# kywind/real2sim-eval

Hardware: AMD Instinct MI355X
Metric: sim env-steps/sec (phys+render) per node at 32 envs (higher is better)
Workload: dtype f32

## Files before the change

### real2sim-eval_amd/csrc/physics_substep.h

```cpp

typedef unsigned v4u __attribute__((ext_vector_type(4)));
constexpr unsigned PF_SENT = 0x7fc5e7a1u;
constexpr int PF_LINE = 128;
constexpr int PF_AUX_STORE = 16;
constexpr int PF_AUX_LOAD = 16 | (int)0x80000000;
__device__ __forceinline__ void resident_fault(const PhysDev& p, int code, int item, int k, unsigned a, unsigned b, unsigned c, unsigned d, unsigned e2, unsigned f)
{
    if (!p.fault) return;
    if (atomicCAS(p.fault, 0, code) == 0) {
        int* w = p.fault + 3;
        w[0] = code; w[1] = item; w[2] = k; w[3] = (int)a; w[4] = (int)b; w[5] = (int)c; w[6] = (int)d; w[7] = (int)e2; w[8] = (int)f;
    }
}
__device__ __forceinline__ bool pf_pending(v2f a) { return __float_as_uint(a.x) == PF_SENT && __float_as_uint(a.y) == PF_SENT; }
__device__ __forceinline__ void pf_mark(StateM s, size_t i)
{
    const v2f w = {__uint_as_float(PF_SENT), __uint_as_float(PF_SENT)};
    s.p[st_at(s.n, i, 0)] = w; s.p[st_at(s.n, i, 1)] = w; s.p[st_at(s.n, i, 2)] = w;
}
__device__ __forceinline__ void pf_store(const PhysDev& p, size_t ei, f3 x, f3 v, unsigned tag)
{
    const __amdgpu_buffer_rsrc_t r = __builtin_amdgcn_make_buffer_rsrc(p.pf_res, 0, 0x7fffffff, 0x00020000);
    const unsigned off = (unsigned)ei * (unsigned)PF_LINE;
    const v4u w0 = {__float_as_uint(x.x), tag, __float_as_uint(x.y), tag}, w1 = {__float_as_uint(x.z), tag, __float_as_uint(v.z), tag},
              w2 = {__float_as_uint(v.x), tag, __float_as_uint(v.y), tag};
    __builtin_amdgcn_raw_buffer_store_b128(w0, r, off, 0, PF_AUX_STORE);
    __builtin_amdgcn_raw_buffer_store_b128(w1, r, off + 16u, 0, PF_AUX_STORE);
    __builtin_amdgcn_raw_buffer_store_b128(w2, r, off + 32u, 0, PF_AUX_STORE);
}
__device__ __forceinline__ void pf_wait(const PhysDev& p, size_t ei, int step, int item, v2f& a, v2f& b, v2f& c)
{
    const __amdgpu_buffer_rsrc_t r = __builtin_amdgcn_make_buffer_rsrc(p.pf_res, 0, 0x7fffffff, 0x00020000);
    const unsigned off = (unsigned)ei * (unsigned)PF_LINE, tag = (unsigned)step;
    for (unsigned spins = 0;; ++spins) {
        const v4u d0 = __builtin_amdgcn_raw_buffer_load_b128(r, off, 0, PF_AUX_LOAD), d1 = __builtin_amdgcn_raw_buffer_load_b128(r, off + 16u, 0, PF_AUX_LOAD),
                  d2 = __builtin_amdgcn_raw_buffer_load_b128(r, off + 32u, 0, PF_AUX_LOAD);
        if (d0.y == tag && d0.w == tag && d1.y == tag && d1.w == tag && d2.y == tag && d2.w == tag) {
            a = (v2f){__uint_as_float(d0.x), __uint_as_float(d0.z)}; b = (v2f){__uint_as_float(d1.x), __uint_as_float(d1.z)};
            c = (v2f){__uint_as_float(d2.x), __uint_as_float(d2.z)};
            return;
        }
        if (spins >= p.spin_limit) {
            resident_fault(p, 6, item, step, (unsigned)ei, d0.y, d0.w, d1.y, d2.y, spins);
            a = (v2f){0.f, 0.f}; b = a; c = a;
            return;
        }
        __builtin_amdgcn_s_sleep(2);
    }
}

#pragma clang fp contract(fast)

__device__ __forceinline__ void spring_term(v2f xy, float zj, v2f vxy, float vzj, f3 xi, f3 vi, float k, float a, float dashpot,
                                            v2f& fxy, float& fz)
{
    const v2f dxy = xy - (v2f){xi.x, xi.y};
    const float dz = zj - xi.z;
    const float d2 = fmaf(dxy.x, dxy.x, fmaf(dxy.y, dxy.y, fmaf(dz, dz, 1e-30f)));
    const float rinv = __builtin_amdgcn_rsqf(d2);
    const v2f dvxy = vxy - (v2f){vi.x, vi.y};
    const float dvz = vzj - vi.z;
    const float t = fmaf(dvxy.x, dxy.x, fmaf(dvxy.y, dxy.y, dvz * dz));
    const float sc = fmaf(dashpot * (rinv * rinv), t, fmaf(-k, rinv, a));
    fxy += dxy * sc;
    fz = fmaf(dz, sc, fz);
}

template <int RCAP> __device__ __forceinline__ constexpr int PLANE1() { return RCAP * 8 + 8; }
template <int RCAP> __device__ __forceinline__ constexpr int PLANE2() { return 2 * (RCAP * 8 + 8); }

struct AdjGroup {
    uint2 idx;
    float4 k, a;
};
__device__ __forceinline__ AdjGroup adj_load(const PhysDev& p, int row, int lane)
{
    typedef unsigned v2u __attribute__((ext_vector_type(2)));
    typedef float v4f __attribute__((ext_vector_type(4)));
    const __amdgpu_buffer_rsrc_t ri = __builtin_amdgcn_make_buffer_rsrc((void*)p.adj_idx, 0, 0x7fffffff, 0x00020000);
    const __amdgpu_buffer_rsrc_t rk = __builtin_amdgcn_make_buffer_rsrc((void*)p.adj_k, 0, 0x7fffffff, 0x00020000);
    const __amdgpu_buffer_rsrc_t ra = __builtin_amdgcn_make_buffer_rsrc((void*)p.adj_ir, 0, 0x7fffffff, 0x00020000);
    const v2u i2 = __builtin_amdgcn_raw_buffer_load_b64(ri, (unsigned)lane * 8u, row * 8, 0);
    const v4f k4 = __builtin_amdgcn_raw_buffer_load_b128(rk, (unsigned)lane * 16u, row * 16, 0);
    const v4f a4 = __builtin_amdgcn_raw_buffer_load_b128(ra, (unsigned)lane * 16u, row * 16, 0);
    AdjGroup g;
    g.idx = make_uint2(i2.x, i2.y); g.k = make_float4(k4.x, k4.y, k4.z, k4.w); g.a = make_float4(a4.x, a4.y, a4.z, a4.w);
    return g;
}

template <int RCAP>
__device__ __forceinline__ void spring_group(const PhysDev& p, const AdjGroup& g, const __attribute__((address_space(3))) char* win, f3 xi,
                                             f3 vi, v2f& fxy, float& fz)
{
    typedef __attribute__((address_space(3))) const v2f lds_f2;
    const unsigned off[GROUP] = {g.idx.x & 0xffffu, g.idx.x >> 16, g.idx.y & 0xffffu, g.idx.y >> 16};
    const float k[GROUP] = {g.k.x, g.k.y, g.k.z, g.k.w};
    const float a[GROUP] = {g.a.x, g.a.y, g.a.z, g.a.w};
#pragma unroll
    for (int u = 0; u < GROUP; ++u) {
#ifdef R2S_WIN16
        typedef float v4f_ __attribute__((ext_vector_type(4)));
        typedef __attribute__((address_space(3))) const v4f_ lds_f4;
        const v4f_ xz = *(lds_f4*)(win + 2u * off[u]);
        const v2f vxy = *(lds_f2*)(win + off[u] + 2 * (RCAP * 8 + 8));
        spring_term((v2f){xz.x, xz.y}, xz.z, vxy, xz.w, xi, vi, k[u], a[u], p.dashpot, fxy, fz);
#else
        const v2f xy = *(lds_f2*)(win + off[u]);
        const v2f zz = *(lds_f2*)(win + off[u] + PLANE1<RCAP>());
        const v2f vxy = *(lds_f2*)(win + off[u] + PLANE2<RCAP>());
        spring_term(xy, zz.x, vxy, zz.y, xi, vi, k[u], a[u], p.dashpot, fxy, fz);
#endif
    }
}

template <int RCAP>
__device__ __forceinline__ f3 spring_force_lds(const PhysDev& p, const StateC xv,
                                               const __attribute__((address_space(3))) char* win, size_t env_base, int sl, int ln, f3 xi,
                                               f3 vi, int srow, int ngroups, AdjGroup g0, int pf_step = -1)
{
    v2f fxy = {0.f, 0.f};
    float fz = 0.f;
    AdjGroup a = g0, b = g0;
    int g = 0;
    for (; g + 2 <= ngroups; g += 2) {
        b = adj_load(p, srow + (g + 1) * SLICE, ln);
        spring_group<RCAP>(p, a, win, xi, vi, fxy, fz);
        a = adj_load(p, srow + min(g + 2, ngroups - 1) * SLICE, ln);
        spring_group<RCAP>(p, b, win, xi, vi, fxy, fz);
    }
    if (g < ngroups) spring_group<RCAP>(p, a, win, xi, vi, fxy, fz);
    const int4* __restrict__ ra = p.radj + p.rslice_off[sl] + ln;
    const int rdeg = p.rslice_deg[sl];
    for (int n = 0; n < rdeg; ++n) {
        const int4 en = ra[n * SLICE];
        const size_t gi = env_base + (size_t)en.x;
        v2f jxy = xv.p[st_at(xv.n, gi, 0)], jz = xv.p[st_at(xv.n, gi, 1)], jv = xv.p[st_at(xv.n, gi, 2)];
        if (pf_step >= 0 && pf_pending(jxy)) pf_wait(p, gi, pf_step, -1, jxy, jz, jv);
        spring_term(jxy, jz.x, jv, jz.y, xi, vi, __int_as_float(en.y), __int_as_float(en.z), p.dashpot, fxy, fz);
    }
    return {fxy.x, fxy.y, fz};
}

#pragma clang fp contract(off)

__device__ __forceinline__ float mesh_margin(const PhysDev& p, int m)
{
    return (p.mesh_kind[m] & 2) ? MESH_MAX_DIST : ((m < p.n_dyn_mesh && !p.use_pusher) ? 0.005f : 0.001f);
}
__device__ __forceinline__ bool mesh_need(const PhysDev& p, int e, int step, f3 next_x, float pad, bool& near, const float* staged = nullptr)
{
    bool need = false;
    near = false;
    for (int m = 0; m < p.n_mesh; ++m) {
        const float* bb = staged ? staged + 6 * m
                        : m < p.n_dyn_mesh ? p.aabb_dyn + (((size_t)e * p.n_sub + step) * p.n_dyn_mesh + m) * 6
                                           : p.aabb_static + ((size_t)e * (p.n_mesh - p.n_dyn_mesh) + (m - p.n_dyn_mesh)) * 6;
        const float mg = mesh_margin(p, m) + pad;
        const float d2 = box_dist2(next_x, bb);
        need = need || d2 < mg * mg * 1.0001f;
        near = near || d2 < (mg + NEAR_PAD) * (mg + NEAR_PAD);
    }
    return need;
}

constexpr int RES_MAX_MESH = 4;
constexpr float RES_RANGE_PAD = 0.002f;
struct ResidentIO {
    bool srv_on, srv_need;
    const float* step_boxes;
    f3 x, v;
    const float* boxes;
};
__device__ __forceinline__ bool resident_in_range(const ResidentIO& io, f3 next_x, bool fin)
{
    if (__builtin_amdgcn_ballot_w64(fin && box_dist2(next_x, io.boxes) < io.boxes[6]) == 0ull) return false;
    bool any = false;
#pragma unroll
    for (int m = 0; m < RES_MAX_MESH; ++m) any = any || box_dist2(next_x, io.boxes + 8 + 8 * m) < io.boxes[8 + 8 * m + 6];
    return __builtin_amdgcn_ballot_w64(fin && any) != 0ull;
}

__device__ __forceinline__ int mesh_rec_reserve(const PhysDev& p, int e, int step)
{
    int slot;
    {
        const unsigned long long act = __builtin_amdgcn_ballot_w64(true);
        const int e0 = __builtin_amdgcn_readfirstlane(e);
        if (__builtin_amdgcn_ballot_w64(e != e0) == 0ull) {
            const int rank = (int)__builtin_amdgcn_mbcnt_hi((unsigned)(act >> 32), __builtin_amdgcn_mbcnt_lo((unsigned)act, 0u));
            int base = 0;
            if (rank == 0) base = atomicAdd(p.rec_cnt + (size_t)e0 * p.n_sub + step, (int)__builtin_popcountll(act));
            slot = __builtin_amdgcn_readfirstlane(base) + rank;
        } else
            slot = atomicAdd(p.rec_cnt + (size_t)e * p.n_sub + step, 1);
    }
    return slot;
}
__device__ __forceinline__ void mesh_rec_write(const PhysDev& p, int e, int step, int slot, int i, int ncand, f3 x0, f3 v)
{
    int4* r = p.mesh_rec + 2 * (par_off(p, step) + (size_t)e * p.N + slot);
    const int hint = p.mq_hint ? p.mq_hint[(size_t)e * p.N + i] : -1;
    r[0] = make_int4(ncand | ((hint + 1) << 19), ncand > 0 ? (i | (int)0x80000000) : i, __float_as_int(x0.x), __float_as_int(x0.y));
    r[1] = make_int4(__float_as_int(x0.z), __float_as_int(v.x), __float_as_int(v.y), __float_as_int(v.z));
}
__device__ __forceinline__ bool mesh_rec_push(const PhysDev& p, int e, int step, int i, int ncand, f3 x0, f3 v)
{
    const int slot = mesh_rec_reserve(p, e, step);
    if (slot >= p.N) return false;
    mesh_rec_write(p, e, step, slot, i, ncand, x0, v);
    return true;
}

template <int MESH, bool MAIN = false, int NEED = 0, bool KEEP = false, bool QUAD = false, bool PFOUT = false>
__device__ __forceinline__ bool finish_wave(const PhysDev& p, int e, int i, size_t eb, int step, int write_forces, f3 x0, f3 v, bool fin,
                                            const StateM xv_out, const TriRegs* tr, QShare* qs, int* qpar, BlkAux* xf0, bool store, ResidentIO* keep R2S_QP_PARAM)
{
    f3 x = x0;
    if (MESH) {
        f3 vin = v;
        f3 next_x = x0 + vin * p.dt;
        f3 next_v = vin;
        bool in_range = true;
        if (KEEP && keep->boxes) in_range = resident_in_range(*keep, next_x, fin);
      if (in_range) {
        bool need = false, near = false;
        if (NEED == 1) need = fin;
        else if (NEED == 0 && fin) need = mesh_need(p, e, step, next_x, 0.f, near, KEEP ? keep->step_boxes : nullptr);
        if (MAIN) {
            const unsigned long long nm = __builtin_amdgcn_ballot_w64(near);
            if (nm && (int)(threadIdx.x & 63) == __builtin_ctzll(nm)) p.mesh_cnt[p.n_sub] = 1;
            const unsigned long long qm = __builtin_amdgcn_ballot_w64(need);
            if (qm && (int)(threadIdx.x & 63) == __builtin_ctzll(qm)) p.fault[1] = 1;
            if (MESH == 2) {
                if (need && mesh_rec_push(p, e, step, i, 0, x0, v)) { fin = false; need = false; }
            } else if (need && p.mesh_defer && p.mesh_rec) {
                if (mesh_rec_push(p, e, step, i, 0, x0, v)) { fin = false; need = false; }
            } else if (need && p.mesh_defer) {
                const int slot = atomicAdd(p.mesh_cnt + step, 1);
                if (slot < p.mesh_cap) {
                    const size_t po = par_off(p, step);
                    p.vdef[po + eb + i] = make_float4(v.x, v.y, v.z, 0.f);
                    p.xbc[po + eb + i] = make_float4(x0.x, x0.y, x0.z, 0.f);
                    p.mesh_list[po + slot] = make_int2(e, i);
                    fin = false;
                    need = false;
                }
            } else if (KEEP && need && keep->srv_on) {
                keep->srv_need = true;
                fin = false;
                need = false;
            }
        }
        constexpr bool IN_PLACE = !(MAIN && MESH == 2) && NEED != 2;
        MeshHit q = {false, 0.f, 0, mk(0.f, 0.f, 0.f), 0, 0};
        if (IN_PLACE)
            q = MESH == 3 ? mesh_query_regs<QUAD>(*tr, mk(bcast(next_x.x, 0), bcast(next_x.y, 0), bcast(next_x.z, 0)), bcasti((int)need, 0) != 0, *qs, *qpar)
              : MESH == 2 ? mesh_query_block(p, step, mk(bcast(next_x.x, 0), bcast(next_x.y, 0), bcast(next_x.z, 0)), e,
                                             bcasti((int)need, 0) != 0, xf0->hint, *qs, *qpar, *xf0 R2S_QP_ARG)
                          : mesh_query_lane(p, e, step, next_x, need);
        R2S_QSTAMP();
        bool requery = false;
        f3 normal = mk(0.f, 0.f, 0.f), v_normal = mk(0.f, 0.f, 0.f), v_normal_new = mk(0.f, 0.f, 0.f);
        float margin = 0.f;
        bool hit = false;
        if (q.result) {
            int is_gripper;
            const int mm = MESH >= 2 ? q.mm : p.mesh_map[q.face];
            if (!p.use_pusher) is_gripper = mm == 0 ? 1 : (mm == 1 ? 2 : 0);
            else is_gripper = mm >= 0 ? 1 : 0;
            f3 delta = next_x - q.pt;
            float dist = len(delta) * q.sign;
            margin = (is_gripper >= 1 && !p.use_pusher) ? 0.005f : 0.001f;
            float err = dist - margin;
            if (err < 0.f) {
                hit = true;
                normal = normalize0(delta) * q.sign;
                f3 rdv = mk(0.f, 0.f, 0.f);
                float ce, cf;
                if (is_gripper >= 1) {
                    const f3 ctr = MESH == 3 ? tr->ctr : ld3(p.interp_center, (size_t)e * p.n_sub + step);
                    const f3 om = MESH == 3 ? tr->om : ld3(p.dyn_omega, e);
                    const f3 dv = MESH == 3 ? (is_gripper == 1 ? tr->dv0 : tr->dv1) : ld3(p.dyn_vel, (size_t)e * 2 + (is_gripper == 1 ? 0 : 1));
                    rdv = dv + cross(om, x0 - ctr);
                    vin = vin - rdv;
                    ce = p.cee; cf = p.cef;
                } else {
                    ce = p.ce; cf = p.cf;
                }
                v_normal = normal * dot(vin, normal);
                const f3 v_tao = vin - v_normal;
                const float vnl = len(v_normal);
                const float vtl = fmaxf(len(v_tao), 1e-6f);
                v_normal_new = v_normal * (-ce);
                const float a = fmaxf(0.f, 1.f - cf * (1.f + ce) * vnl / vtl);
                next_v = v_normal_new + v_tao * a;
                if (is_gripper >= 1) {
                    next_v = next_v + rdv;
                    next_x = x0 + next_v * p.dt;
                    requery = true;
                } else {
                    next_x = next_x - normal * err;
                }
            }
        }
        MeshHit q2 = {false, 0.f, 0, mk(0.f, 0.f, 0.f), 0, 0};
        if (IN_PLACE)
            q2 = MESH == 3 ? mesh_query_regs<QUAD>(*tr, mk(bcast(next_x.x, 0), bcast(next_x.y, 0), bcast(next_x.z, 0)), bcasti((int)requery, 0) != 0, *qs, *qpar)
               : MESH == 2 ? mesh_query_block(p, step, mk(bcast(next_x.x, 0), bcast(next_x.y, 0), bcast(next_x.z, 0)), e,
                                              bcasti((int)requery, 0) != 0, bcasti(q.hint, 0), *qs, *qpar, *xf0 R2S_QP_ARG)
                           : mesh_query_lane(p, e, step, next_x, requery);
        R2S_QSTAMP();
        if (requery) {
            if (q2.result) {
                const f3 delta = next_x - q2.pt;
                const float dist = len(delta) * q2.sign;
                const float err = dist - margin;
                if (err < 0.f) {
                    normal = normalize0(delta) * q2.sign;
                    next_x = next_x - normal * err;
                }
            }
            q = q2;
        }
        if (MESH == 2 && IN_PLACE && !MAIN && fin && store && p.mq_hint) p.mq_hint[eb + i] = q.hint;
        if (hit && write_forces && store) {
            const f3 fo = (v_normal_new - v_normal) / p.dt;
            float* cf3 = p.coll_forces + ((size_t)e * p.nF + (MESH >= 2 ? q.fm : p.face_map[q.face])) * 3;
            atomicAdd(cf3, fo.x);
            atomicAdd(cf3 + 1, fo.y);
            atomicAdd(cf3 + 2, fo.z);
            atomicAdd(p.hit_cnt + e, 1);
        }
      }
        x = next_x;
        v = next_v;
    }

    if (fin && (store || KEEP)) {
        const f3 normal = mk(0.f, 0.f, 1.f) * p.rf;
        const float x_z = x.z, v_z = v.z;
        const float next_x_z = (x_z + v_z * p.dt) * p.rf;
        f3 v1;
        float toi;
        if (next_x_z < 0.f && v_z * p.rf < -1e-4f) {
            const f3 v_normal = normal * dot(v, normal);
            const f3 v_tao = v - v_normal;
            const float vnl = len(v_normal);
            const float vtl = fmaxf(len(v_tao), 1e-6f);
            const f3 v_normal_new = v_normal * (-p.ce);
            const float a = fmaxf(0.f, 1.f - p.cf * (1.f + p.ce) * vnl / vtl);
            v1 = v_normal_new + v_tao * a;
            toi = -(x_z - 0.f) / v_z;
        } else {
            v1 = v;
            toi = 0.f;
        }
        const f3 xn = x + v * toi + v1 * (p.dt - toi);
        if (PFOUT) { if (store) pf_store(p, eb + (size_t)i, xn, v1, (unsigned)step + 1u); }
        else if (store && (!KEEP || xv_out.p != nullptr)) st_store(xv_out, eb + i, xn, v1);
        if (KEEP) { keep->x = xn; keep->v = v1; }
        return true;
    }
    return false;
}

#ifdef R2S_PHASE_PROBE
__device__ long long g_phase_probe[8192 * 4];
#define R2S_STAMP(k) do { if (threadIdx.x == 0 && blockIdx.x < 8192) g_phase_probe[blockIdx.x * 4 + (k)] = (long long)wall_clock64(); } while (0)
extern "C" int r2s_phys_debug_phase_probe(long long* out, int n)
{
    return (int)hipMemcpyFromSymbol(out, HIP_SYMBOL(g_phase_probe), sizeof(long long) * (size_t)n * 4);
}
#else
#define R2S_STAMP(k) do { } while (0)
#endif

template <int B, int RCAP, bool SELF, int MESH, bool PF = false, bool EXTWIN = false>
__device__ __forceinline__ void substep_body(const PhysDev& p, const StateC xv_in, const StateM xv_out, int step,
                                             int write_forces, int bid, __attribute__((address_space(3))) v2f* win_ext = nullptr)
{
    static_assert(B % SLICE == 0 && RCAP >= B && RCAP * 8 <= 65536, "window offsets are u16 bytes");
    __shared__ __attribute__((aligned(16))) v2f win_own[EXTWIN ? 1 : 3 * (RCAP + 1)];
    __attribute__((address_space(3))) v2f* const win_s = EXTWIN ? win_ext : (__attribute__((address_space(3))) v2f*)win_own;
    const int xcd = bid & 7, q = bid >> 3;
    const int item = xcd * p.cb + q;
    if (q >= p.cb || item >= p.nb * p.ne) return;
#ifndef R2S_NO_SCALAR_ENV
    const int b = __builtin_amdgcn_readfirstlane(item / p.ne), e = __builtin_amdgcn_readfirstlane(p.e0 + (item - b * p.ne));
#else
    const int b = item / p.ne, e = p.e0 + (item - b * p.ne);
#endif
    R2S_STAMP(0);
    const int tid = threadIdx.x;
    const int lane = tid & 63;
    const int i = b * B + tid;
    const bool valid = i < p.N;
    const size_t eb = (size_t)e * p.N;
    const int ic = min(i, p.N - 1);
    const int sl = __builtin_amdgcn_readfirstlane(ic / SLICE);
    const int srow = __builtin_amdgcn_readfirstlane(p.slice_off[sl] / GROUP);
    const int ngroups = __builtin_amdgcn_readfirstlane(p.slice_deg[sl] / GROUP);
    AdjGroup g0;
    g0.idx = make_uint2(0u, 0u); g0.k = make_float4(0.f, 0.f, 0.f, 0.f); g0.a = g0.k;
    if (ngroups > 0) g0 = adj_load(p, srow, lane);
    constexpr int K = (RCAP + B - 1) / B;
#ifndef R2S_STAGE_BATCH
#define R2S_STAGE_BATCH 4
#endif
#ifndef R2S_STAGE64
#define R2S_STAGE64 2
#endif
    constexpr int KB = B == 64 ? (R2S_STAGE64 < K ? R2S_STAGE64 : K) : ((R2S_STAGE_BATCH > 0 && R2S_STAGE_BATCH < K) ? R2S_STAGE_BATCH : K);
    const int h0 = p.halo_off[b], per_env = B + (p.halo_off[b + 1] - h0);
    v2f own_a = {0.f, 0.f}, own_b = own_a, own_c = own_a;
#pragma unroll
    for (int k0 = 0; k0 < K; k0 += KB) {
        int part[KB];
#pragma unroll
        for (int k = 0; k < KB; ++k) {
            const int r = tid + (k0 + k) * B;
            part[k] = (k0 + k >= K) ? p.N : (r < B ? i : (r < per_env ? p.halo_ids[h0 + r - B] : p.N));
        }
        v2f qa[KB], qb[KB], qc[KB];
#pragma unroll
        for (int k = 0; k < KB; ++k) {
            const size_t g = eb + (size_t)min(part[k], p.N - 1);
            if (part[k] < p.N) { qa[k] = xv_in.p[st_at(xv_in.n, g, 0)]; qb[k] = xv_in.p[st_at(xv_in.n, g, 1)]; qc[k] = xv_in.p[st_at(xv_in.n, g, 2)]; }
            else { qa[k] = (v2f){0.f, 0.f}; qb[k] = qa[k]; qc[k] = qa[k]; }
        }
        if (PF) {
#pragma unroll
            for (int k = 0; k < KB; ++k)
                if (part[k] < p.N && pf_pending(qa[k])) pf_wait(p, eb + (size_t)part[k], step, item, qa[k], qb[k], qc[k]);
        }
#pragma unroll
        for (int k = 0; k < KB; ++k) {
            const int r = tid + (k0 + k) * B;
            if (r < RCAP && part[k] < p.N) {
#ifdef R2S_WIN16
                win_s[2 * r] = qa[k];
                win_s[2 * r + 1] = qb[k];
                win_s[2 * (RCAP + 1) + r] = qc[k];
#else
                win_s[r] = qa[k];
                win_s[RCAP + 1 + r] = qb[k];
                win_s[2 * (RCAP + 1) + r] = qc[k];
#endif
            }
        }
        if (k0 == 0) { own_a = qa[0]; own_b = qb[0]; own_c = qc[0]; }
    }
    __syncthreads();
    R2S_STAMP(1);
    const f3 x0 = mk(own_a.x, own_a.y, own_b.x), v0 = mk(own_c.x, own_c.y, own_b.y);
    const float m1 = p.masses[ic];

    const __attribute__((address_space(3))) char* win = (const __attribute__((address_space(3))) char*)win_s;
    f3 v = vel_update(p, v0, spring_force_lds<RCAP>(p, xv_in, win, eb, sl, lane, x0, v0, srow, ngroups, g0, PF ? step : -1), m1);
#ifdef R2S_PHASE_PROBE
    if (v.x == 1.2345e33f) return;
#endif
    R2S_STAMP(2);

    bool fin = valid;
    const bool rec_mode = PF && MESH != 0 && p.mesh_rec != nullptr && (p.mesh_defer || MESH == 2);
    int tag_ncand = 0;
    if (SELF) {
        const int ncand = valid ? p.coll_num[eb + i] : 0;
        if (ncand > 0) {
            const size_t po = par_off(p, step);
            p.vbc[po + eb + i] = make_float4(v.x, v.y, v.z, 0.f);
            p.xbc[po + eb + i] = make_float4(x0.x, x0.y, x0.z, 0.f);
            fin = false;
            if (rec_mode) tag_ncand = ncand;
            else if (MESH != 0 && (p.mesh_defer || MESH == 2)) {
                bool near;
                if (mesh_need(p, e, step, x0 + v * p.dt, 0.002f, near)) {
                    p.fault[1] = 1;
                    if (MESH == 2 || p.mesh_rec) {
                        if (mesh_rec_push(p, e, step, i, ncand, x0, v)) p.cand_mark[po + eb + i] = step + 1;
                    } else {
                        const int slot = atomicAdd(p.mesh_cnt + step, 1);
                        if (slot < p.mesh_cap) {
                            p.mesh_list[po + slot] = make_int2(e | (ncand << 12), i | (int)0x80000000);
                            p.cand_mark[po + eb + i] = step + 1;
                        }
                    }
                }
                const unsigned long long nm = __builtin_amdgcn_ballot_w64(near);
                if (nm && lane == __builtin_ctzll(nm)) p.mesh_cnt[p.n_sub] = 1;
            }
        }
    }
    R2S_QP_DECL(-1);
    bool done;
    if (rec_mode) {
        bool near = false, need = false;
        if (fin || tag_ncand > 0) need = mesh_need(p, e, step, x0 + v * p.dt, tag_ncand > 0 ? 0.002f : 0.f, near);
        const unsigned long long nm = __builtin_amdgcn_ballot_w64(near);
        if (nm && lane == __builtin_ctzll(nm)) p.mesh_cnt[p.n_sub] = 1;
        const unsigned long long qm = __builtin_amdgcn_ballot_w64(need);
        if (qm && lane == __builtin_ctzll(qm)) p.fault[1] = 1;
        int slot = 0;
        if (need) { slot = mesh_rec_reserve(p, e, step); fin = false; }
        done = finish_wave<MESH, false, 2>(p, e, i, eb, step, write_forces, x0, v, fin, xv_out, nullptr, nullptr, nullptr, nullptr, true, nullptr R2S_QP_ARG);
        if (need) {
            if (slot < p.N) {
                mesh_rec_write(p, e, step, slot, i, tag_ncand, x0, v);
                if (tag_ncand > 0) p.cand_mark[par_off(p, step) + eb + i] = step + 1;
            } else
                resident_fault(p, 8, item, step, (unsigned)(eb + i), (unsigned)slot, 0u, 0u, 0u, 0u);
        }
    } else
        done = finish_wave<MESH, MESH != 0>(p, e, i, eb, step, write_forces, x0, v, fin, xv_out, nullptr, nullptr, nullptr, nullptr, true, nullptr R2S_QP_ARG);
    if (PF && valid && !done) pf_mark(xv_out, eb + i);
    R2S_STAMP(3);
}

template <int B, int RCAP, bool SELF, int MESH>
__global__ void __launch_bounds__(B, (B == 256 ? 6 : 1)) k_substep(const PhysDev p, const StateC xv_in, const StateM xv_out, int step,
                                               int write_forces)
{
    substep_body<B, RCAP, SELF, MESH>(p, xv_in, xv_out, step, write_forces, (int)blockIdx.x);
}
```

### real2sim-eval_amd/csrc/physics.hip

```cpp

#include "r2s_common.h"
#include <rocprim/rocprim.hpp>
#include "../../include/r2s_physics.h"
#include "physics_flavour.h"
#include <algorithm>
#include <array>
#include <climits>
#include <cmath>
#include <cstdlib>
#include <mutex>
#include <vector>
#include <functional>

namespace {

constexpr int SLICE = 64;

constexpr int GROUP = 4;
constexpr int TPB = 256;
constexpr int GRID_DIM = 128;
constexpr int GRID_CELL_BITS = 21;
constexpr float MESH_MAX_DIST = 0.02f;
constexpr float WIND_THRESHOLD = 0.6f;
constexpr float NEAR_PAD = 0.03f;
// ... 596 lines not shown

struct ResidentGate {
    std::mutex mu;
    hipEvent_t last[16] = {};
    bool recorded[16] = {};
};
ResidentGate& resident_gate() { static ResidentGate g; return g; }
int resident_enter(hipStream_t s, int* dev_out)
{
    int dev = 0;
    R2S_HIP_TRY(hipGetDevice(&dev));
    if (dev < 0 || dev >= 16) return R2S_ERR_INVALID;
    ResidentGate& g = resident_gate();
    g.mu.lock();
    if (g.recorded[dev]) {
        const hipError_t e = hipStreamWaitEvent(s, g.last[dev], 0);
        if (e != hipSuccess) { g.mu.unlock(); R2S_HIP_TRY(e); }
    }
    *dev_out = dev;
    return R2S_OK;
}
int resident_leave(hipStream_t s, int dev)
{
    ResidentGate& g = resident_gate();
    hipError_t e = hipSuccess;
    if (!g.last[dev]) e = hipEventCreateWithFlags(&g.last[dev], hipEventDisableTiming);
    if (e == hipSuccess) e = hipEventRecord(g.last[dev], s);
    if (e == hipSuccess) g.recorded[dev] = true;
    g.mu.unlock();
    R2S_HIP_TRY(e);
    return R2S_OK;
}

int launch_graphs(R2SPhys* h, int slot, hipStream_t s)
{
    const int chains = h->chains();
    if (chains > 1) {
        if (!h->chain_fork) R2S_HIP_TRY(hipEventCreateWithFlags(&h->chain_fork, hipEventDisableTiming));
        R2S_HIP_TRY(hipEventRecord(h->chain_fork, s));
    }
    for (int c = 1; c < chains; ++c) {
        hipStream_t sc = chain_side_stream(c);
        if (!sc) return R2S_ERR_HIP;
        if (!h->chain_join[c]) R2S_HIP_TRY(hipEventCreateWithFlags(&h->chain_join[c], hipEventDisableTiming));
        R2S_HIP_TRY(hipStreamWaitEvent(sc, h->chain_fork, 0));
        R2S_HIP_TRY(hipGraphLaunch(h->graph_exec[c][slot], sc));
    }
    R2S_HIP_TRY(hipGraphLaunch(h->graph_exec[0][slot], s));
    for (int c = 1; c < chains; ++c) {
        hipStream_t sc = chain_side_stream(c);
        if (h->graph_exec_tail[c][slot]) R2S_HIP_TRY(hipGraphLaunch(h->graph_exec_tail[c][slot], sc));
        R2S_HIP_TRY(hipEventRecord(h->chain_join[c], sc));
    }
    if (h->graph_exec_tail[0][slot]) R2S_HIP_TRY(hipGraphLaunch(h->graph_exec_tail[0][slot], s));
    for (int c = 1; c < chains; ++c) R2S_HIP_TRY(hipStreamWaitEvent(s, h->chain_join[c], 0));
    return R2S_OK;
}

int resolve_cand_count(R2SPhys* h)
{
    if (h->cand_pending) {
        R2S_HIP_TRY(hipEventSynchronize(h->cand_event));
        h->n_cand = *h->h_cand_count;
        h->cand_pending = false;
    }
    return R2S_OK;
}

int update_mesh_transforms(R2SPhys* h, hipStream_t s)
{
    if (h->n_xf == 0) return R2S_OK;
    const int tot = h->E * h->prm.num_substeps * h->n_xf;
    R2S_HIP_TRY(hipMemsetAsync(h->d_rigid_err, 0, sizeof(unsigned), s));
    hipLaunchKernelGGL(k_mesh_xf, dim3((tot + 255) / 256), dim3(256), 0, s, h->E, h->prm.num_substeps, h->n_dyn_mesh, h->n_dyn_pts, h->n_xf, h->d_xf_mesh,
                       h->d_xf_ref, h->d_mesh_vert_off, h->d_rest_pts, h->d_xf_rest_box, h->d_interp, h->d_xf, h->d_aabb_dyn, h->d_rigid_err);
    R2S_HIP_TRY(hipMemcpyAsync(h->h_rigid_err, h->d_rigid_err, sizeof(unsigned), hipMemcpyDeviceToHost, s));
    if (!h->rigid_event) R2S_HIP_TRY(hipEventCreateWithFlags(&h->rigid_event, hipEventDisableTiming));
    R2S_HIP_TRY(hipEventRecord(h->rigid_event, s));
    h->rigid_pending = true;
    R2S_HIP_TRY(hipGetLastError());
    return R2S_OK;
}

__global__ void __launch_bounds__(256) k_tri_pre(const PhysDev p, float4* __restrict__ out)
{
    const size_t t = (size_t)blockIdx.x * blockDim.x + threadIdx.x;
    const size_t tot = (size_t)p.E * p.n_sub * p.nF;
    if (t >= tot) return;
    const int f = (int)(t % p.nF);
    const size_t es = t / p.nF;
    const int e = (int)(es / p.n_sub), step = (int)(es % p.n_sub);
    const f3 a = mesh_vertex(p, e, step, p.faces[3 * f]), b = mesh_vertex(p, e, step, p.faces[3 * f + 1]), c = mesh_vertex(p, e, step, p.faces[3 * f + 2]);
    int m = 0;
    for (int k = 1; k < p.n_mesh; ++k) m += f >= p.mesh_face_off[k] ? 1 : 0;
    float4* o = out + es * 5 * p.nF + f;
    o[0] = make_float4(a.x, a.y, a.z, b.x);
    o[(size_t)p.nF] = make_float4(b.y, b.z, c.x, c.y);
    o[(size_t)2 * p.nF] = make_float4(c.z, __int_as_float(p.mesh_map[f]), __int_as_float(p.face_map[f]), __int_as_float(m));
    o[(size_t)3 * p.nF] = make_float4(fminf(a.x, fminf(b.x, c.x)), fminf(a.y, fminf(b.y, c.y)), fminf(a.z, fminf(b.z, c.z)), fmaxf(a.x, fmaxf(b.x, c.x)));
    o[(size_t)4 * p.nF] = make_float4(fmaxf(a.y, fmaxf(b.y, c.y)), fmaxf(a.z, fmaxf(b.z, c.z)), 0.f, 0.f);
}
void update_tri_pre(R2SPhys* h, hipStream_t s)
{
    if (!h->d_tri_pre) return;
    const size_t tot = (size_t)h->E * h->prm.num_substeps * h->nF;
    hipLaunchKernelGGL(k_tri_pre, dim3((unsigned)((tot + 255) / 256)), dim3(256), 0, s, h->dev(), h->d_tri_pre);
}

int grid_sort(R2SPhys* h, hipStream_t s, const uint32_t** keys, const uint32_t** ids, bool fine = false)
{
    const float cell = h->prm.collision_dist * 5.0f;
    const float cell_inv = 1.0f / cell;
    dim3 grid((h->N + TPB - 1) / TPB, h->E);
    if (fine) hipLaunchKernelGGL(k_fine_keys, grid, dim3(TPB), 0, s, h->N, h->E, h->state(h->cur), 1.0f / h->prm.collision_dist, h->d_keys[0], h->d_ids[0]);
    else hipLaunchKernelGGL(k_grid_keys, grid, dim3(TPB), 0, s, h->N, h->E, h->d_inv, h->state(h->cur), cell_inv, h->d_keys[0], h->d_ids[0]);
    rocprim::double_buffer<uint32_t> dk(h->d_keys[0], h->d_keys[1]);
    rocprim::double_buffer<uint32_t> dv(h->d_ids[0], h->d_ids[1]);
    unsigned bits = GRID_CELL_BITS;
    while ((1u << (bits - GRID_CELL_BITS)) < (unsigned)h->E) ++bits;
    size_t need = h->sort_bytes;
    R2S_HIP_TRY(rocprim::radix_sort_pairs(h->d_sort_tmp, need, dk, dv, (size_t)h->E * h->N, 0u, bits, s));
    *keys = dk.current();
    *ids = dv.current();
    return R2S_OK;
}

void report_fault(const int* cnt)
{
    if (cnt[1] >= 2 && cnt[1] <= 7) {
        char buf[640];
        const int* w = cnt + 4;
        snprintf(buf, sizeof buf, "resident stepper: a workgroup waited for %s beyond the poll limit (the launch was not resident at once, or the device "
                 "is shared with a kernel that never ends); the state is invalid [first fault: code %d, work item %d, substep %d of the launch, context %d %d %d %d %d %d]",
                 cnt[1] == 2 ? "a neighbour block's substep" : cnt[1] == 5 ? "a neighbour's record (server pair)" : cnt[1] == 6 ? "a particle finished by the head of its launch" : cnt[1] == 7 ? "a self-collision partner's record" : "a mesh-query server's result", w[0], w[1], w[2], w[3], w[4], w[5], w[6], w[7], w[8]);
        r2s::set_last_error_msg(buf);
    } else if (cnt[1] == 8) {
        r2s::set_last_error_msg("a per-environment list of particles left to the finishing code overflowed (more than N entries in one substep: cannot happen in a sound launch); the state is invalid");
    } else
        r2s::set_last_error_msg("a self-collision impulse changed a particle's velocity by more than 40 m/s within one substep: its mesh-contact "
                                "test (widened by 2 mm) may have been skipped where the reference applies it (unsupported)");
}

}

extern "C" {

int r2s_phys_create(const R2SPhysDesc* d, R2SPhys** out, r2s_stream_t stream_)
{
    hipStream_t s = (hipStream_t)stream_;
    if (!d || !out || d->n_env <= 0 || d->num_object_points <= 0 || d->num_springs < 0 || !d->init_vertices || !d->init_masses ||
        (d->num_springs > 0 && (!d->init_springs || !d->init_rest_lengths || !d->init_spring_Y)) || d->params.num_substeps <= 0)
        return R2S_ERR_INVALID;
    if ((uint64_t)d->n_env >= (1u << (32 - GRID_CELL_BITS))) return R2S_ERR_INVALID;
    R2SPhys* h = new (std::nothrow) R2SPhys();
    if (!h) return R2S_ERR_ALLOC;
    h->prm = d->params;
    h->E = d->n_env; h->N = d->num_object_points; h->S = d->num_springs;
    h->coll_cap = d->collision_capacity > 0 ? d->collision_capacity : 500;
    if (h->coll_cap >= (1 << 19)) { delete h; return R2S_ERR_INVALID; }
    const int N = h->N, E = h->E, S = h->S;
    for (int sp = 0; sp < S; ++sp)
        if (d->init_springs[2 * sp] < 0 || d->init_springs[2 * sp] >= N || d->init_springs[2 * sp + 1] < 0 || d->init_springs[2 * sp + 1] >= N) {
            delete h; return R2S_ERR_INVALID;
        }
    h->h_springs.assign(d->init_springs, d->init_springs + 2 * (size_t)S);
    h->h_rest.assign(d->init_rest_lengths, d->init_rest_lengths + S);
    int rc = R2S_OK;
#define TRY(x) do { rc = (x); if (rc != R2S_OK) { r2s_phys_destroy(h); return rc; } } while (0)

    {
        const int sizes[3] = {256, 128, 64}, caps[3] = {1024, 768, 512};
        int pick = 0;
        if (const char* ev = getenv("R2S_RESIDENT")) h->resident_pref = atoi(ev) != 0;
        if (h->resident_pref && (int64_t)((h->N + 63) / 64) * h->E <= RES_MAX_ITEMS) pick = 2;
        if (const char* ev = getenv("R2S_LAYOUT")) { const int v = atoi(ev); for (int k = 0; k < 3; ++k) if (v == sizes[k]) pick = k; }
        h->pb = sizes[pick]; h->rcap = caps[pick];
        if (const char* ev = getenv("R2S_CHAINS")) h->chains_override = atoi(ev);
        if (const char* ev = getenv("R2S_GRAPH_HEAD")) h->graph_head = std::max(0, atoi(ev));
        if (const char* ev = getenv("R2S_MESH_DEFER")) h->force_defer = atoi(ev) != 0;
    }
    const int PB = h->pb, SL = SLICE;
    h->h_perm.resize(N); h->h_inv.resize(N);
    {
        float lo[3] = {3e38f, 3e38f, 3e38f}, hi[3] = {-3e38f, -3e38f, -3e38f};
        for (int i = 0; i < N; ++i)
            for (int k = 0; k < 3; ++k) { lo[k] = std::min(lo[k], d->init_vertices[3 * i + k]); hi[k] = std::max(hi[k], d->init_vertices[3 * i + k]); }
        const float ext = std::max(std::max(hi[0] - lo[0], hi[1] - lo[1]), std::max(hi[2] - lo[2], 1e-9f));
        auto spread = [](uint64_t v) {
            v &= 0x1fffff; v = (v | v << 32) & 0x1f00000000ffffull; v = (v | v << 16) & 0x1f0000ff0000ffull;
            v = (v | v << 8) & 0x100f00f00f00f00full; v = (v | v << 4) & 0x10c30c30c30c30c3ull; v = (v | v << 2) & 0x1249249249249249ull;
            return v;
        };
        std::vector<std::pair<uint64_t, int>> code(N);
        for (int i = 0; i < N; ++i) {
            uint64_t c = 0;
            for (int k = 0; k < 3; ++k) {
                const double t = (d->init_vertices[3 * i + k] - lo[k]) / ext;
                c |= spread((uint64_t)std::min(1048575.0, std::max(0.0, t * 1048575.0))) << k;
            }
            code[i] = {c, i};
        }
        std::sort(code.begin(), code.end());
        std::vector<int> degree(N, 0);
        for (int sp = 0; sp < S; ++sp) { degree[h->h_springs[2 * sp]]++; degree[h->h_springs[2 * sp + 1]]++; }
        for (int b0 = 0; b0 < N; b0 += PB)
            std::stable_sort(code.begin() + b0, code.begin() + std::min(N, b0 + PB),
                             [&](const std::pair<uint64_t, int>& a, const std::pair<uint64_t, int>& b) { return degree[a.second] > degree[b.second]; });
        for (int i = 0; i < N; ++i) { h->h_perm[i] = code[i].second; h->h_inv[code[i].second] = i; }
    }
    TRY(dev_alloc(&h->d_perm, N)); TRY(dev_alloc(&h->d_inv, N));
    TRY(upload(h->d_perm, h->h_perm.data(), N, s)); TRY(upload(h->d_inv, h->h_inv.data(), N, s));

    std::vector<std::vector<std::pair<int, int>>> adj(N);
    for (int sp = 0; sp < S; ++sp) {
        const int a = h->h_inv[h->h_springs[2 * sp]], b = h->h_inv[h->h_springs[2 * sp + 1]];
        adj[a].push_back({b, sp});
        adj[b].push_back({a, sp});
    }
    for (auto& l : adj) std::sort(l.begin(), l.end());
    h->n_slices = (N + SL - 1) / SL;
    h->nb = (N + PB - 1) / PB;
    h->cb = (h->nb * E + 7) / 8;
    int HALO_CAP = h->rcap - PB;
    if (const char* ev = getenv("R2S_HALO_CAP")) HALO_CAP = std::min(HALO_CAP, std::max(0, atoi(ev)));
    std::vector<int> halo_off(h->nb + 1, 0), halo_ids;
    std::vector<int> slot_of(N, -1);
    std::vector<std::vector<int>> halo_of_block(h->nb);
    h->halo_max = 0;
    for (int b = 0; b < h->nb; ++b) {
        std::vector<std::pair<int, int>> cnt;
        {
            std::vector<int> refs;
            for (int i = b * PB; i < std::min(N, (b + 1) * PB); ++i)
                for (auto& nb : adj[i]) if (nb.first / PB != b) refs.push_back(nb.first);
            std::sort(refs.begin(), refs.end());
            for (size_t a = 0; a < refs.size();) {
                size_t e2 = a;
                while (e2 < refs.size() && refs[e2] == refs[a]) ++e2;
                cnt.push_back({-(int)(e2 - a), refs[a]});
                a = e2;
            }
        }
        std::sort(cnt.begin(), cnt.end());
        if ((int)cnt.size() > HALO_CAP) cnt.resize(HALO_CAP);
        std::vector<int>& hl = halo_of_block[b];
        for (auto& c : cnt) hl.push_back(c.second);
        std::sort(hl.begin(), hl.end());
        halo_off[b + 1] = halo_off[b] + (int)hl.size();
        halo_ids.insert(halo_ids.end(), hl.begin(), hl.end());
        h->halo_max = std::max(h->halo_max, (int)hl.size());
    }
    std::vector<std::vector<std::array<int, 3>>> loc(N), rem(N);
    for (int b = 0; b < h->nb; ++b) {
        const std::vector<int>& hl = halo_of_block[b];
        for (size_t k = 0; k < hl.size(); ++k) slot_of[hl[k]] = PB + (int)k;
        for (int i = b * PB; i < std::min(N, (b + 1) * PB); ++i)
            for (auto& nb : adj[i]) {
                const int j = nb.first;
                if (j / PB == b) loc[i].push_back({j, nb.second, j % PB});
                else if (slot_of[j] >= 0) loc[i].push_back({j, nb.second, slot_of[j]});
                else rem[i].push_back({j, nb.second, -1});
            }
        for (size_t k = 0; k < hl.size(); ++k) slot_of[hl[k]] = -1;
    }
    h->h_slice_int.assign(h->n_slices, 0);
    if (PB == SL)
        for (int b = 0; b < h->nb; ++b) {
            int imax = 0;
            for (int i = b * PB; i < std::min(N, (b + 1) * PB); ++i) {
                std::stable_partition(loc[i].begin(), loc[i].end(), [&](const std::array<int, 3>& a) { return a[2] < PB; });
                int ni = 0;
                for (auto& a : loc[i]) ni += a[2] < PB;
                imax = std::max(imax, ni);
            }
            imax = (imax + GROUP - 1) / GROUP * GROUP;
            h->h_slice_int[b] = imax;
            for (int i = b * PB; i < std::min(N, (b + 1) * PB); ++i) {
                int ni = 0;
                for (auto& a : loc[i]) ni += a[2] < PB;
                loc[i].insert(loc[i].begin() + ni, (size_t)(imax - ni), std::array<int, 3>{i, -1, i % PB});
            }
        }
    auto build_ell = [&](const std::vector<std::vector<std::array<int, 3>>>& lists, std::vector<int>& off, std::vector<int>& deg,
                         std::vector<int>& a_spring, std::vector<int>& a_nbr, std::vector<int>& a_self, std::vector<int>* a_loc) {
        off.assign(h->n_slices, 0); deg.assign(h->n_slices, 0);
        int total = 0;
        for (int sl = 0; sl < h->n_slices; ++sl) {
            int dmax = 0;
            for (int i = sl * SL; i < std::min(N, (sl + 1) * SL); ++i) dmax = std::max(dmax, (int)lists[i].size());
            dmax = (dmax + GROUP - 1) / GROUP * GROUP;
            off[sl] = total; deg[sl] = dmax;
            total += dmax * SL;
        }
        a_spring.assign(total, -1); a_nbr.assign(total, 0); a_self.assign(total, 0);
        if (a_loc) a_loc->assign(total, 0);
        for (int sl = 0; sl < h->n_slices; ++sl)
            for (int ln = 0; ln < SL; ++ln) {
                const int i = sl * SL + ln;
                const int self = i < N ? i : (i / PB) * PB;
                for (int n = 0; n < deg[sl]; ++n) {
                    const int t = off[sl] + n * SL + ln;
                    a_self[t] = self;
                    if (a_loc) (*a_loc)[t] = self % PB;
                    if (i < N && n < (int)lists[i].size()) {
                        a_nbr[t] = lists[i][n][0]; a_spring[t] = lists[i][n][1];
                        if (a_loc) (*a_loc)[t] = lists[i][n][2];
// ... 1082 lines not shown
```

Baseline: 1848.

## Software-pipeline LDS neighbor reads one slot ahead in spring force loop

Splits the adjacency load into separate index and stiffness/rest-length loads, and prefetches index rows two groups ahead. Each LDS neighbor record is read one spring ahead of its use, with sched_barriers keeping the read ahead of the current spring's arithmetic. The aim is to hide LDS and global load latency behind the spring math. In exchange it raises register pressure, adds an explicit waitcnt, and the sched_barriers limit how freely the compiler can schedule.

```diff
diff --git a/real2sim-eval_amd/csrc/physics_substep.h b/real2sim-eval_amd/csrc/physics_substep.h
--- a/real2sim-eval_amd/csrc/physics_substep.h
+++ b/real2sim-eval_amd/csrc/physics_substep.h
@@ -87,48 +87,111 @@
     g.idx = make_uint2(i2.x, i2.y); g.k = make_float4(k4.x, k4.y, k4.z, k4.w); g.a = make_float4(a4.x, a4.y, a4.z, a4.w);
     return g;
 }
+struct AdjKA { float4 k, a; };
+__device__ __forceinline__ uint2 adj_load_idx(const PhysDev& p, int row, int lane)
+{
+    typedef unsigned v2u __attribute__((ext_vector_type(2)));
+    const __amdgpu_buffer_rsrc_t ri = __builtin_amdgcn_make_buffer_rsrc((void*)p.adj_idx, 0, 0x7fffffff, 0x00020000);
+    const v2u i2 = __builtin_amdgcn_raw_buffer_load_b64(ri, (unsigned)lane * 8u, row * 8, 0);
+    return make_uint2(i2.x, i2.y);
+}
+__device__ __forceinline__ AdjKA adj_load_ka(const PhysDev& p, int row, int lane)
+{
+    typedef float v4f __attribute__((ext_vector_type(4)));
+    const __amdgpu_buffer_rsrc_t rk = __builtin_amdgcn_make_buffer_rsrc((void*)p.adj_k, 0, 0x7fffffff, 0x00020000);
+    const __amdgpu_buffer_rsrc_t ra = __builtin_amdgcn_make_buffer_rsrc((void*)p.adj_ir, 0, 0x7fffffff, 0x00020000);
+    const v4f k4 = __builtin_amdgcn_raw_buffer_load_b128(rk, (unsigned)lane * 16u, row * 16, 0);
+    const v4f a4 = __builtin_amdgcn_raw_buffer_load_b128(ra, (unsigned)lane * 16u, row * 16, 0);
+    AdjKA g;
+    g.k = make_float4(k4.x, k4.y, k4.z, k4.w); g.a = make_float4(a4.x, a4.y, a4.z, a4.w);
+    return g;
+}
+struct AdjHead { uint2 i0, i1; AdjKA ka; };
+__device__ __forceinline__ AdjHead adj_head(const PhysDev& p, int srow, int ngroups, int lane)
+{
+    AdjHead h;
+    h.i0 = adj_load_idx(p, srow, lane);
+    h.i1 = adj_load_idx(p, srow + min(1, ngroups - 1) * SLICE, lane);
+    h.ka = adj_load_ka(p, srow, lane);
+    return h;
+}
+
+#ifdef R2S_WIN16
+typedef float v4f_win16 __attribute__((ext_vector_type(4)));
+struct SlotRec { v4f_win16 xz; v2f vxy; };
+template <int RCAP> __device__ __forceinline__ SlotRec slot_read(const __attribute__((address_space(3))) char* win, unsigned off)
+{
+    typedef __attribute__((address_space(3))) const v2f lds_f2;
+    typedef __attribute__((address_space(3))) const v4f_win16 lds_f4;
+    SlotRec r;
+    r.xz = *(lds_f4*)(win + 2u * off);
+    r.vxy = *(lds_f2*)(win + off + 2 * (RCAP * 8 + 8));
+    return r;
+}
+__device__ __forceinline__ void slot_term(const SlotRec& r, f3 xi, f3 vi, float k, float a, float dashpot, v2f& fxy, float& fz)
+{
+    spring_term((v2f){r.xz.x, r.xz.y}, r.xz.z, r.vxy, r.xz.w, xi, vi, k, a, dashpot, fxy, fz);
+}
+#else
+struct SlotRec { v2f xy, zz, vxy; };
+template <int RCAP> __device__ __forceinline__ SlotRec slot_read(const __attribute__((address_space(3))) char* win, unsigned off)
+{
+    typedef __attribute__((address_space(3))) const v2f lds_f2;
+    SlotRec r;
+    r.xy = *(lds_f2*)(win + off);
+    r.zz = *(lds_f2*)(win + off + PLANE1<RCAP>());
+    r.vxy = *(lds_f2*)(win + off + PLANE2<RCAP>());
+    return r;
+}
+__device__ __forceinline__ void slot_term(const SlotRec& r, f3 xi, f3 vi, float k, float a, float dashpot, v2f& fxy, float& fz)
+{
+    spring_term(r.xy, r.zz.x, r.vxy, r.zz.y, xi, vi, k, a, dashpot, fxy, fz);
+}
+#endif
 
 template <int RCAP>
-__device__ __forceinline__ void spring_group(const PhysDev& p, const AdjGroup& g, const __attribute__((address_space(3))) char* win, f3 xi,
-                                             f3 vi, v2f& fxy, float& fz)
-{
-    typedef __attribute__((address_space(3))) const v2f lds_f2;
-    const unsigned off[GROUP] = {g.idx.x & 0xffffu, g.idx.x >> 16, g.idx.y & 0xffffu, g.idx.y >> 16};
+__device__ __forceinline__ void spring_group(const PhysDev& p, uint2 idx, const AdjKA& g, unsigned next_off, const __attribute__((address_space(3))) char* win,
+                                             f3 xi, f3 vi, SlotRec& cur, v2f& fxy, float& fz)
+{
     const float k[GROUP] = {g.k.x, g.k.y, g.k.z, g.k.w};
     const float a[GROUP] = {g.a.x, g.a.y, g.a.z, g.a.w};
 #pragma unroll
     for (int u = 0; u < GROUP; ++u) {
-#ifdef R2S_WIN16
-        typedef float v4f_ __attribute__((ext_vector_type(4)));
-        typedef __attribute__((address_space(3))) const v4f_ lds_f4;
-        const v4f_ xz = *(lds_f4*)(win + 2u * off[u]);
-        const v2f vxy = *(lds_f2*)(win + off[u] + 2 * (RCAP * 8 + 8));
-        spring_term((v2f){xz.x, xz.y}, xz.z, vxy, xz.w, xi, vi, k[u], a[u], p.dashpot, fxy, fz);
-#else
-        const v2f xy = *(lds_f2*)(win + off[u]);
-        const v2f zz = *(lds_f2*)(win + off[u] + PLANE1<RCAP>());
-        const v2f vxy = *(lds_f2*)(win + off[u] + PLANE2<RCAP>());
-        spring_term(xy, zz.x, vxy, zz.y, xi, vi, k[u], a[u], p.dashpot, fxy, fz);
-#endif
+        const unsigned off = u == 0 ? idx.x >> 16 : u == 1 ? idx.y & 0xffffu : u == 2 ? idx.y >> 16 : next_off;
+        const SlotRec nxt = slot_read<RCAP>(win, off);
+        __builtin_amdgcn_sched_barrier(0);
+        slot_term(cur, xi, vi, k[u], a[u], p.dashpot, fxy, fz);
+        __builtin_amdgcn_sched_barrier(0);
+        cur = nxt;
     }
 }
 
 template <int RCAP>
 __device__ __forceinline__ f3 spring_force_lds(const PhysDev& p, const StateC xv,
                                                const __attribute__((address_space(3))) char* win, size_t env_base, int sl, int ln, f3 xi,
-                                               f3 vi, int srow, int ngroups, AdjGroup g0, int pf_step = -1)
-{
+                                               f3 vi, int srow, int ngroups, AdjHead h, int pf_step = -1)
+{
+    static_assert(GROUP == 4, "spring_group names the four offsets of a group");
     v2f fxy = {0.f, 0.f};
     float fz = 0.f;
-    AdjGroup a = g0, b = g0;
-    int g = 0;
-    for (; g + 2 <= ngroups; g += 2) {
-        b = adj_load(p, srow + (g + 1) * SLICE, ln);
-        spring_group<RCAP>(p, a, win, xi, vi, fxy, fz);
-        a = adj_load(p, srow + min(g + 2, ngroups - 1) * SLICE, ln);
-        spring_group<RCAP>(p, b, win, xi, vi, fxy, fz);
-    }
-    if (g < ngroups) spring_group<RCAP>(p, a, win, xi, vi, fxy, fz);
+    if (ngroups > 0) {
+        uint2 ia = h.i0, ib = h.i1;
+        AdjKA ka = h.ka, kb = h.ka;
+        const int last = ngroups - 1;
+        SlotRec cur = slot_read<RCAP>(win, ia.x & 0xffffu);
+        __builtin_amdgcn_s_waitcnt(0xc07f);
+        int g = 0;
+        for (; g + 2 <= ngroups; g += 2) {
+            kb = adj_load_ka(p, srow + (g + 1) * SLICE, ln);
+            const uint2 ic = adj_load_idx(p, srow + min(g + 2, last) * SLICE, ln);
+            spring_group<RCAP>(p, ia, ka, ib.x & 0xffffu, win, xi, vi, cur, fxy, fz);
+            ka = adj_load_ka(p, srow + min(g + 2, last) * SLICE, ln);
+            const uint2 id = adj_load_idx(p, srow + min(g + 3, last) * SLICE, ln);
+            spring_group<RCAP>(p, ib, kb, ic.x & 0xffffu, win, xi, vi, cur, fxy, fz);
+            ia = ic; ib = id;
+        }
+        if (g < ngroups) spring_group<RCAP>(p, ia, ka, ia.x & 0xffffu, win, xi, vi, cur, fxy, fz);
+    }
     const int4* __restrict__ ra = p.radj + p.rslice_off[sl] + ln;
     const int rdeg = p.rslice_deg[sl];
     for (int n = 0; n < rdeg; ++n) {
@@ -400,9 +463,9 @@
     const int sl = __builtin_amdgcn_readfirstlane(ic / SLICE);
     const int srow = __builtin_amdgcn_readfirstlane(p.slice_off[sl] / GROUP);
     const int ngroups = __builtin_amdgcn_readfirstlane(p.slice_deg[sl] / GROUP);
-    AdjGroup g0;
-    g0.idx = make_uint2(0u, 0u); g0.k = make_float4(0.f, 0.f, 0.f, 0.f); g0.a = g0.k;
-    if (ngroups > 0) g0 = adj_load(p, srow, lane);
+    AdjHead g0;
+    g0.i0 = make_uint2(0u, 0u); g0.i1 = g0.i0; g0.ka.k = make_float4(0.f, 0.f, 0.f, 0.f); g0.ka.a = g0.ka.k;
+    if (ngroups > 0) g0 = adj_head(p, srow, ngroups, lane);
     constexpr int K = (RCAP + B - 1) / B;
 #ifndef R2S_STAGE_BATCH
 #define R2S_STAGE_BATCH 4
```

Result: no change. 1854 (median of 2 runs) (+0.3%).

## Batch halo staging loads and pending-flag waits in substep prologue

Applied to the files above, without the earlier changes.

Moves computation of the first batch of halo particle ids ahead of the adjacency load so the index loads issue earlier. State records are now loaded through a buffer resource as one 128-bit plus one 64-bit load per particle, guarded by a wave ballot instead of a per-lane branch. The adjacency load becomes unconditional, using an out-of-bounds offset to yield zeros when a slice has no groups. The per-particle spin wait on prefetch flags is replaced by a staged wait that polls all pending slots in one loop. A size check guards the 32-bit byte offsets, and lanes with no data may now be left uninitialised where the old code wrote zeros.

```diff
diff --git a/real2sim-eval_amd/csrc/physics.hip b/real2sim-eval_amd/csrc/physics.hip
--- a/real2sim-eval_amd/csrc/physics.hip
+++ b/real2sim-eval_amd/csrc/physics.hip
@@ -772,6 +772,7 @@
         (d->num_springs > 0 && (!d->init_springs || !d->init_rest_lengths || !d->init_spring_Y)) || d->params.num_substeps <= 0)
         return R2S_ERR_INVALID;
     if ((uint64_t)d->n_env >= (1u << (32 - GRID_CELL_BITS))) return R2S_ERR_INVALID;
+    if ((uint64_t)d->num_object_points * 24u >= (1ull << 31)) return R2S_ERR_INVALID;
     R2SPhys* h = new (std::nothrow) R2SPhys();
     if (!h) return R2S_ERR_ALLOC;
     h->prm = d->params;
diff --git a/real2sim-eval_amd/csrc/physics_substep.h b/real2sim-eval_amd/csrc/physics_substep.h
--- a/real2sim-eval_amd/csrc/physics_substep.h
+++ b/real2sim-eval_amd/csrc/physics_substep.h
@@ -46,6 +46,33 @@
             return;
         }
         __builtin_amdgcn_s_sleep(2);
+    }
+}
+template <int KB>
+__device__ __forceinline__ void pf_wait_staged(const PhysDev& p, size_t eb, const int (&part)[KB], unsigned pend, int step, int item, v2f (&a)[KB],
+                                               v2f (&b)[KB], v2f (&c)[KB])
+{
+    const __amdgpu_buffer_rsrc_t r = __builtin_amdgcn_make_buffer_rsrc(p.pf_res, 0, 0x7fffffff, 0x00020000);
+    const unsigned tag = (unsigned)step;
+    for (unsigned spins = 0; pend != 0u; ++spins) {
+#pragma unroll
+        for (int k = 0; k < KB; ++k) {
+            if (!(pend & (1u << k))) continue;
+            const size_t ei = eb + (size_t)part[k];
+            const unsigned off = (unsigned)ei * (unsigned)PF_LINE;
+            const v4u d0 = __builtin_amdgcn_raw_buffer_load_b128(r, off, 0, PF_AUX_LOAD), d1 = __builtin_amdgcn_raw_buffer_load_b128(r, off + 16u, 0, PF_AUX_LOAD),
+                      d2 = __builtin_amdgcn_raw_buffer_load_b128(r, off + 32u, 0, PF_AUX_LOAD);
+            if (d0.y == tag && d0.w == tag && d1.y == tag && d1.w == tag && d2.y == tag && d2.w == tag) {
+                a[k] = (v2f){__uint_as_float(d0.x), __uint_as_float(d0.z)}; b[k] = (v2f){__uint_as_float(d1.x), __uint_as_float(d1.z)};
+                c[k] = (v2f){__uint_as_float(d2.x), __uint_as_float(d2.z)};
+                pend &= ~(1u << k);
+            } else if (spins >= p.spin_limit) {
+                resident_fault(p, 6, item, step, (unsigned)ei, d0.y, d0.w, d1.y, d2.y, spins);
+                a[k] = (v2f){0.f, 0.f}; b[k] = a[k]; c[k] = a[k];
+                pend &= ~(1u << k);
+            }
+        }
+        if (pend != 0u) __builtin_amdgcn_s_sleep(2);
     }
 }
 
@@ -73,16 +100,16 @@
     uint2 idx;
     float4 k, a;
 };
-__device__ __forceinline__ AdjGroup adj_load(const PhysDev& p, int row, int lane)
+__device__ __forceinline__ AdjGroup adj_load(const PhysDev& p, int row, int lane, unsigned oob = 0u)
 {
     typedef unsigned v2u __attribute__((ext_vector_type(2)));
     typedef float v4f __attribute__((ext_vector_type(4)));
     const __amdgpu_buffer_rsrc_t ri = __builtin_amdgcn_make_buffer_rsrc((void*)p.adj_idx, 0, 0x7fffffff, 0x00020000);
     const __amdgpu_buffer_rsrc_t rk = __builtin_amdgcn_make_buffer_rsrc((void*)p.adj_k, 0, 0x7fffffff, 0x00020000);
     const __amdgpu_buffer_rsrc_t ra = __builtin_amdgcn_make_buffer_rsrc((void*)p.adj_ir, 0, 0x7fffffff, 0x00020000);
-    const v2u i2 = __builtin_amdgcn_raw_buffer_load_b64(ri, (unsigned)lane * 8u, row * 8, 0);
-    const v4f k4 = __builtin_amdgcn_raw_buffer_load_b128(rk, (unsigned)lane * 16u, row * 16, 0);
-    const v4f a4 = __builtin_amdgcn_raw_buffer_load_b128(ra, (unsigned)lane * 16u, row * 16, 0);
+    const v2u i2 = __builtin_amdgcn_raw_buffer_load_b64(ri, ((unsigned)lane * 8u) | oob, row * 8, 0);
+    const v4f k4 = __builtin_amdgcn_raw_buffer_load_b128(rk, ((unsigned)lane * 16u) | oob, row * 16, 0);
+    const v4f a4 = __builtin_amdgcn_raw_buffer_load_b128(ra, ((unsigned)lane * 16u) | oob, row * 16, 0);
     AdjGroup g;
     g.idx = make_uint2(i2.x, i2.y); g.k = make_float4(k4.x, k4.y, k4.z, k4.w); g.a = make_float4(a4.x, a4.y, a4.z, a4.w);
     return g;
@@ -375,6 +402,27 @@
 #define R2S_STAMP(k) do { } while (0)
 #endif
 
+#ifndef R2S_STAGE_BATCH
+#define R2S_STAGE_BATCH 4
+#endif
+#ifndef R2S_STAGE64
+#define R2S_STAGE64 2
+#endif
+__device__ __forceinline__ void st_load_rec(const StateC s, size_t eb, int id, v2f& a, v2f& b, v2f& c)
+{
+#ifdef R2S_STATE_PLANES
+    const size_t g = eb + (size_t)id;
+    a = s.p[st_at(s.n, g, 0)]; b = s.p[st_at(s.n, g, 1)]; c = s.p[st_at(s.n, g, 2)];
+#else
+    typedef float v4f __attribute__((ext_vector_type(4)));
+    const __amdgpu_buffer_rsrc_t rs = __builtin_amdgcn_make_buffer_rsrc((void*)(s.p + 3 * eb), 0, 0x7fffffff, 0x00020000);
+    const unsigned off = (unsigned)id * 24u;
+    const v4f ab = __builtin_amdgcn_raw_buffer_load_b128(rs, off, 0, 0);
+    const v2f cc = __builtin_amdgcn_raw_buffer_load_b64(rs, off + 16u, 0, 0);
+    a = (v2f){ab.x, ab.y}; b = (v2f){ab.z, ab.w}; c = cc;
+#endif
+}
+
 template <int B, int RCAP, bool SELF, int MESH, bool PF = false, bool EXTWIN = false>
 __device__ __forceinline__ void substep_body(const PhysDev& p, const StateC xv_in, const StateM xv_out, int step,
                                              int write_forces, int bid, __attribute__((address_space(3))) v2f* win_ext = nullptr)
@@ -397,21 +445,25 @@
     const bool valid = i < p.N;
     const size_t eb = (size_t)e * p.N;
     const int ic = min(i, p.N - 1);
+    constexpr int K = (RCAP + B - 1) / B;
+    constexpr int KB = B == 64 ? (R2S_STAGE64 < K ? R2S_STAGE64 : K) : ((R2S_STAGE_BATCH > 0 && R2S_STAGE_BATCH < K) ? R2S_STAGE_BATCH : K);
+    const int h0 = p.halo_off[b], per_env = B + (p.halo_off[b + 1] - h0);
+    int part0[KB];
+#pragma unroll
+    for (int k = 0; k < KB; ++k) {
+        const int r = tid + k * B;
+        part0[k] = (k >= K) ? p.N : (r < B ? i : (r < per_env ? p.halo_ids[h0 + r - B] : p.N));
+    }
     const int sl = __builtin_amdgcn_readfirstlane(ic / SLICE);
     const int srow = __builtin_amdgcn_readfirstlane(p.slice_off[sl] / GROUP);
     const int ngroups = __builtin_amdgcn_readfirstlane(p.slice_deg[sl] / GROUP);
     AdjGroup g0;
-    g0.idx = make_uint2(0u, 0u); g0.k = make_float4(0.f, 0.f, 0.f, 0.f); g0.a = g0.k;
-    if (ngroups > 0) g0 = adj_load(p, srow, lane);
-    constexpr int K = (RCAP + B - 1) / B;
-#ifndef R2S_STAGE_BATCH
-#define R2S_STAGE_BATCH 4
-#endif
-#ifndef R2S_STAGE64
-#define R2S_STAGE64 2
-#endif
-    constexpr int KB = B == 64 ? (R2S_STAGE64 < K ? R2S_STAGE64 : K) : ((R2S_STAGE_BATCH > 0 && R2S_STAGE_BATCH < K) ? R2S_STAGE_BATCH : K);
-    const int h0 = p.halo_off[b], per_env = B + (p.halo_off[b + 1] - h0);
+    if (PF) {
+        g0.idx = make_uint2(0u, 0u); g0.k = make_float4(0.f, 0.f, 0.f, 0.f); g0.a = g0.k;
+        if (ngroups > 0) g0 = adj_load(p, srow, lane);
+    } else
+        g0 = adj_load(p, ngroups > 0 ? srow : 0, lane, ngroups > 0 ? 0u : 0x80000000u);
+    const size_t ebu = (size_t)__builtin_amdgcn_readfirstlane(e) * p.N;
     v2f own_a = {0.f, 0.f}, own_b = own_a, own_c = own_a;
 #pragma unroll
     for (int k0 = 0; k0 < K; k0 += KB) {
@@ -419,19 +471,18 @@
 #pragma unroll
         for (int k = 0; k < KB; ++k) {
             const int r = tid + (k0 + k) * B;
-            part[k] = (k0 + k >= K) ? p.N : (r < B ? i : (r < per_env ? p.halo_ids[h0 + r - B] : p.N));
+            part[k] = k0 == 0 ? part0[k] : (k0 + k >= K) ? p.N : (r < B ? i : (r < per_env ? p.halo_ids[h0 + r - B] : p.N));
         }
         v2f qa[KB], qb[KB], qc[KB];
 #pragma unroll
-        for (int k = 0; k < KB; ++k) {
-            const size_t g = eb + (size_t)min(part[k], p.N - 1);
-            if (part[k] < p.N) { qa[k] = xv_in.p[st_at(xv_in.n, g, 0)]; qb[k] = xv_in.p[st_at(xv_in.n, g, 1)]; qc[k] = xv_in.p[st_at(xv_in.n, g, 2)]; }
-            else { qa[k] = (v2f){0.f, 0.f}; qb[k] = qa[k]; qc[k] = qa[k]; }
-        }
+        for (int k = 0; k < KB; ++k)
+            if (__builtin_amdgcn_ballot_w64(part[k] < p.N) != 0ull) st_load_rec(xv_in, ebu, min(part[k], p.N - 1), qa[k], qb[k], qc[k]);
         if (PF) {
+            unsigned pend = 0u;
 #pragma unroll
             for (int k = 0; k < KB; ++k)
-                if (part[k] < p.N && pf_pending(qa[k])) pf_wait(p, eb + (size_t)part[k], step, item, qa[k], qb[k], qc[k]);
+                if (part[k] < p.N && pf_pending(qa[k])) pend |= 1u << k;
+            if (pend) pf_wait_staged<KB>(p, eb, part, pend, step, item, qa, qb, qc);
         }
 #pragma unroll
         for (int k = 0; k < KB; ++k) {
@@ -448,7 +499,7 @@
 #endif
             }
         }
-        if (k0 == 0) { own_a = qa[0]; own_b = qb[0]; own_c = qc[0]; }
+        if (k0 == 0 && valid) { own_a = qa[0]; own_b = qb[0]; own_c = qc[0]; }
     }
     __syncthreads();
     R2S_STAMP(1);
```

Measured after the change: 1840 before, 1859 after (median of 6 runs). 1.01x the previous value.
